# wangbaonan/RAG-SNVBERT

Hardware: AMD Instinct MI355X
Metric: masked SNVs imputed/sec (+ kNN queries/sec), window=1024 k=32 (higher is better)
Workload: dtype bf16

## Files before the change

### include/snvrag.h

```cpp
#ifndef SNVRAG_H
#define SNVRAG_H

#include <stddef.h>
#include <stdint.h>

#ifdef __cplusplus
extern "C" {
#endif

#define SNVRAG_ABI_VERSION 31

enum { SNVRAG_F32 = 0, SNVRAG_BF16 = 1 };
enum { SNVRAG_ACT_NONE = 0, SNVRAG_ACT_GELU = 1, SNVRAG_ACT_LRELU = 2, SNVRAG_ACT_SIGMOID = 3 };

int snvrag_abi_version(void);
const char* snvrag_last_error(void);
int snvrag_device_info(int device, char* name, int name_len);
int snvrag_set_option(const char* name, int64_t value);
int snvrag_get_option(const char* name, int64_t* value);

typedef struct {
  const float* bias;
  const float* row1; int64_t row1_stride; const float* col1;
  const float* row2; int64_t row2_stride; const float* col2;
// ... 61 lines not shown
} snvrag_afgate_w_t;
int snvrag_af_gate(int dtype_out, int64_t M, int64_t D, const float* af, const float* af_p,
                   const snvrag_afgate_w_t* w, void* out, void* stream);

int snvrag_rag_weighted_concat(int dtype, int64_t M, int64_t D, const void* q, const void* rag,
                               const void* wgt, int64_t period, void* out, void* stream);

int snvrag_hap_head_out(int dtype_in, int64_t M, int64_t K, const void* H, int64_t ldh,
                        const float* w , const float* b ,
                        float* logits , float* probs , void* stream);
typedef struct {
  const float* f_w; const float* f_b;
  const float* n_w; const float* n_b;
  const float* w1; const float* b1;
  const float* ln_w; const float* ln_b;
  const float* w2; const float* b2;
  const float* c_w; const float* c_b;
} snvrag_gt_w_t;
int snvrag_gt_head(int64_t M, const float* p1, const float* p2, const float* ref,
                   const float* het, const float* hom, int64_t period,
                   const snvrag_gt_w_t* w, float* out , void* stream);

size_t snvrag_knn_lut_bytes(int64_t nq, int32_t n_sites_pad, int limbs);
int snvrag_knn_lut(int64_t nq, int64_t L, int64_t D, const int64_t* tok_q, const float* W,
                   const float* Aq, int64_t aq_period, const float* Ar,
                   const uint8_t* site_mask, int32_t n_sites, int32_t n_sites_pad,
                   int tok0, int tok1, int mask_tok, int limbs,
                   void* lut_out, int32_t* exp_out, float* const_out, void* stream);
int snvrag_knn_lut_panel(int64_t nq, int64_t L, int64_t D, const int64_t* tok_q, const float* W,
                         const float* Wp, const float* Aq, int64_t aq_period, const float* Ar,
                         const uint8_t* site_mask, int32_t n_sites, int32_t n_sites_pad,
                         int tok0, int tok1, int mask_tok, int limbs,
                         void* lut_out, int32_t* exp_out, float* const_out, void* stream);

int snvrag_knn_scan_parts(int64_t n_ref, int32_t nq);
int snvrag_knn_scan(const uint8_t* codes, int64_t n_ref, int64_t ld_codes, int32_t n_sites_pad,
                    const void* lut, int32_t nq, int limbs, int k, int64_t ref_offset,
                    uint64_t* part_keys, int32_t n_parts, const int32_t* th_init, void* stream);
int snvrag_knn_threshold(const uint64_t* keys, int32_t nq, int k, int32_t* th_out, void* stream);
size_t snvrag_topk_merge_ws_bytes(int32_t n_lists, int32_t nq, int k);
int snvrag_topk_merge(const uint64_t* keys, int32_t n_lists, int32_t nq, int k,
                      uint64_t* out_keys, void* ws, size_t ws_bytes, void* stream);
int snvrag_knn_decode(const uint64_t* keys, int32_t nq, int k, const int32_t* exps,
                      const float* consts, int64_t* idx_out, float* dist_out, void* stream);

int snvrag_knn_emb_splits(int64_t N, int64_t K, int Bq);
size_t snvrag_knn_emb_ws_bytes(int64_t N, int Bq, int splits);
size_t snvrag_knn_emb_packed_bytes(int64_t N, int64_t K);
int snvrag_knn_emb_pack(const void* E, int64_t N, int64_t K, void* Et, void* stream);
int snvrag_knn_emb_scan(const void* Et, int64_t N, int64_t K, const void* Q, int Bq, int splits, float* ws,
                        void* stream);
int snvrag_knn_emb_finish(const float* ws, int splits, int Bq, int64_t N, const float* qn, const float* rn,
                          float* dist, void* stream);

int snvrag_rag_mean(int dtype_out, int64_t nq, int64_t L, int64_t D, int k, const int64_t* idx,
                    const uint8_t* codes, int64_t ld_codes, int32_t n_sites,
                    const float* W, const float* pe, const float* Ar,
                    int tok0, int tok1, int sos, int eos, int pad, void* out, void* stream);

int snvrag_neighbor_counts(int64_t nq, int k, const int64_t* idx, const uint8_t* codes, int64_t ld,
                           int64_t row0, int64_t n_rows, uint8_t* counts, int64_t ld_out, void* stream);
int snvrag_rag_mean_counts(int dtype_out, int64_t nq, int64_t L, int64_t D, int k, const int64_t* idx,
                           const uint8_t* counts, int64_t ld_counts, int32_t n_sites,
                           const float* W, const float* pe, const float* Ar,
                           int tok0, int tok1, int sos, int eos, int pad, void* out, void* stream);

// ... 250 lines not shown
```

### rag-snvbert_amd/csrc/common.h

```cpp
#pragma once
#include <hip/hip_runtime.h>
#include <stdint.h>
#include <stddef.h>
#include <string>
#include <type_traits>

#pragma clang diagnostic ignored "-Winline-asm"

#include "../../include/snvrag.h"
#include "host.h"

namespace snvrag {

typedef __bf16 bf16;
typedef __bf16 bf16x8 __attribute__((ext_vector_type(8)));
typedef __bf16 bf16x4 __attribute__((ext_vector_type(4)));
typedef float f32x4 __attribute__((ext_vector_type(4)));
typedef float f32x16 __attribute__((ext_vector_type(16)));
typedef int i32x4 __attribute__((ext_vector_type(4)));
typedef uint32_t u32x4 __attribute__((ext_vector_type(4)));

void set_error(const std::string& msg);

enum EvKind { EV_GEMM = 1, EV_ATTN = 2, EV_LN = 3, EV_KNN_SCAN = 4, EV_KNN_LUT = 5, EV_MERGE = 6, EV_OTHER = 7, EV_BLOCK = 8,
              EV_ATTN_BWD = 10, EV_TRAIN = 11 };
bool evlog_on();
void evlog_begin(hipStream_t s);
void evlog_end(hipStream_t s, int kind, double work);
struct Options {
  int64_t knn_no_reduce;
  int64_t scan_mode;
  int64_t scan_nt;
  int64_t unfused_ln;
  int64_t encoder_chunk;
  int64_t gemm_tile128;
  int64_t gemm_nw;
  int64_t tail_variant;
  int64_t tail_desync;
  int64_t sg_desync;
  int64_t mlp_desync;
  int64_t g2_desync;
  int64_t sg_waves4;
  int64_t ln_bwd_nopf;
  int64_t attn_variant;
  int64_t dw_xcd;
  int64_t ln_rows1;
  int64_t g2_groups;
  int64_t g2_variant;
  int64_t tail_split;
  int64_t proj_wide;
  int64_t tail_wide;
  int64_t tail_qkv;
  int64_t deterministic;
};
Options& options();
unsigned long long* diag_stamps();

int tailw_launch(int M, const void* att, const void* resid, void* out, const void* ws, const float* vec,
                 const float* b_o, const float* g1, const float* be1, float eps, int desync, int var,
                 const void* pw, const float* pbias, void* qkv_out, hipStream_t s);

int projw_launch(int M, int NC, const void* x, const void* ws, const float* bias, void* out, int desync, hipStream_t s);

// ... 95 lines not shown
```

### rag-snvbert_amd/csrc/knn.hip

```cpp
#include "common.h"

namespace snvrag {

constexpr uint64_t KEY_MAX = ~0ull;
constexpr int KEY_BIAS = 1 << 30;
constexpr int SCAN_CAP = 64;
constexpr int SCAN_TH = SCAN_CAP - 16;

__device__ __forceinline__ uint64_t make_key(int d, uint32_t idx) {
  return ((uint64_t)(uint32_t)(d + KEY_BIAS) << 32) | idx;
}

__device__ __forceinline__ int gcd_u(int a, int b) {
  uint32_t x = (uint32_t)a, y = (uint32_t)b;
  while (y) { const uint32_t t = x % y; x = y; y = t; }
  return (int)x;
}

constexpr int LUT_CH = 64;
__host__ __device__ inline int lut_nch_max(int n_sites_pad) { return 2 * n_sites_pad / LUT_CH + 4; }

__global__ __launch_bounds__(256) void lut_delta_kernel(int L, int D, const int64_t* __restrict__ tok_q,
                                                        const float* __restrict__ W, const float* __restrict__ Wp,
                                                        const float* __restrict__ Aq,
// ... 532 lines not shown
  }
}

__global__ void panel_pack_bits_kernel(const uint8_t* __restrict__ codes, long n, long ld, uint8_t* __restrict__ bits,
                                       long ldb) {
  const long chunks_per_row = ldb / 2;
  const long id = (long)blockIdx.x * blockDim.x + threadIdx.x;
  if (id >= n * chunks_per_row) return;
  const long r = id / chunks_per_row;
  const long c0 = (id % chunks_per_row) * 16;
  uint32_t w = 0;
  if (c0 < ld) {
    const u32x4 v = *reinterpret_cast<const u32x4*>(codes + r * ld + c0);
#pragma unroll
    for (int j = 0; j < 16; ++j) w |= ((v[j >> 2] >> (8 * (j & 3))) & 1u) << j;
  }
  *reinterpret_cast<uint16_t*>(bits + r * ldb + c0 / 8) = (uint16_t)w;
}

__global__ void panel_unpack_rows_kernel(const uint8_t* __restrict__ bits, long n_ref, long ldb,
                                         const int64_t* __restrict__ rows, long n_rows, uint8_t* __restrict__ out,
                                         long ld_out) {
  const long chunks_per_row = ld_out / 16;
  const long id = (long)blockIdx.x * blockDim.x + threadIdx.x;
  if (id >= n_rows * chunks_per_row) return;
  const long i = id / chunks_per_row;
  const long c0 = (id % chunks_per_row) * 16;
  const long r = rows[i];
  u32x4 v = u32x4{0, 0, 0, 0};
  if (r >= 0 && r < n_ref && c0 < 8 * ldb) v = expand16(*reinterpret_cast<const uint16_t*>(bits + r * ldb + c0 / 8));
  *reinterpret_cast<u32x4*>(out + i * ld_out + c0) = v;
}

constexpr int S2_CAP = 64;
constexpr int S2_TH = S2_CAP - 16;
constexpr int S2_LDS = 160 * 1024;
constexpr int S2_CAND = 8 * 16 * S2_CAP * 8;
__host__ __device__ constexpr int s2_rows(int KS) { return 32; }
__host__ __device__ constexpr int s2_nst(int KS) {
  return (S2_LDS - S2_CAND) / (s2_rows(KS) * KS * 64) > 3 ? 3 : (S2_LDS - S2_CAND) / (s2_rows(KS) * KS * 64);
}

template <int PPW, int V>
__device__ __forceinline__ void vm_wait_stages(int y) {
  if constexpr (V <= 0) {
    asm volatile("s_waitcnt vmcnt(0)" ::: "memory");
  } else {
    if (y >= V) {
      asm volatile("s_waitcnt vmcnt(%0)" ::"n"(PPW * V) : "memory");
      return;
    }
    vm_wait_stages<PPW, V - 1>(y);
  }
}
typedef uint32_t u32x2 __attribute__((ext_vector_type(2)));
constexpr int S2B_PD = 3;
#ifndef S2_QTW1
#define S2_QTW1 1
#endif

__device__ __forceinline__ void compact_row2(uint64_t* buf, int row, int cnt, int k, int lane, int& new_cnt,
                                             int& new_th) {
  uint64_t key = lane < cnt ? buf[row * S2_CAP + lane] : KEY_MAX;
  key = wave_sort64(key, lane);
  if (lane < k) buf[row * S2_CAP + lane] = key;
  new_cnt = cnt < k ? cnt : k;
// ... 289 lines not shown
                                    const float* Wp, const float* Aq, int64_t aq_period, const float* Ar,
                                    const uint8_t* site_mask, int32_t n_sites, int32_t n_sites_pad, int tok0,
                                    int tok1, int mask_tok, int limbs, void* lut_out, int32_t* exp_out,
                                    float* const_out, void* stream) {
  SNV_CHECK_PTRS(tok_q, W, Wp, site_mask, lut_out, exp_out);
  SNV_CHECK_ARG(limbs == 1 || limbs == 2, "limbs must be 1 or 2");
  SNV_CHECK_ARG(n_sites_pad % 64 == 0 && n_sites_pad >= n_sites && n_sites + 2 <= L, "site padding");
  SNV_CHECK_ARG(n_sites_pad <= 20 * 64, "window longer than 1280 sites");
  if (nq == 0) return 0;
  hipStream_t s = as_stream(stream);
  const size_t sh = (size_t)(n_sites_pad + 4) * sizeof(float);
  if (limbs == 2) {
    char* tail = (char*)lut_out + lut_tail_offset(nq, n_sites_pad);
    SNV_HIP(hipMemsetAsync(tail, 0, (size_t)((nq + 15) / 16) * 16 * 4 + 16, s));
  }
  float* gdelta = (float*)((char*)lut_out + lut_ws_offset(nq, n_sites_pad, limbs));
  float* gcpart = gdelta + (size_t)nq * n_sites_pad;
  if (Aq || Ar) {
    SNV_CHECK_ARG(D % 4 == 0 && aligned(16, W, Wp, Aq, Ar),
                  "offset LUT: D % 4 == 0 and 16-byte aligned W / Wp / Aq / Ar (float4 rows)");
    const int64_t nch = std::min<int64_t>((L + LUT_CH - 1) / LUT_CH, lut_nch_max(n_sites_pad));
    hipLaunchKernelGGL(lut_delta_kernel, dim3((unsigned)nch, (unsigned)nq), dim3(256), 0, s,
                       (int)L, (int)D, tok_q, W, Wp, Aq, (long)aq_period, Ar, site_mask, n_sites, n_sites_pad, tok0,
                       tok1, mask_tok, gdelta, gcpart);
    SNV_LAUNCH_CHECK();
  }
  hipLaunchKernelGGL(lut_kernel, dim3((unsigned)nq), dim3(256), sh, s, (int)L, (int)D, tok_q, W, Wp, Aq,
                     (long)aq_period, Ar, site_mask, n_sites, n_sites_pad, (int)nq, tok0, tok1, mask_tok,
                     limbs, (int8_t*)lut_out, exp_out, const_out, gdelta, gcpart);
  SNV_LAUNCH_CHECK();
  if (nq % 16)
    hipLaunchKernelGGL(lut_zero_pad_kernel, dim3(64), dim3(256), 0, s, (int8_t*)lut_out, (int)nq,
                       n_sites_pad / 64, limbs);
  SNV_LAUNCH_CHECK();
  return 0;
}

__global__ void threshold_kernel(const uint64_t* __restrict__ keys, int nq, int k, int* __restrict__ th) {
  const int q = blockIdx.x * blockDim.x + threadIdx.x;
  if (q >= nq) return;
  const uint64_t key = keys[(long)q * k + k - 1];
  th[q] = key == KEY_MAX ? INT_MAX : (int)(key >> 32) - KEY_BIAS + 1;
}

extern "C" int snvrag_knn_threshold(const uint64_t* keys, int32_t nq, int k, int32_t* th_out, void* stream) {
  SNV_CHECK_ARG(keys && th_out && k >= 1, "bad arguments");
  if (nq == 0) return 0;
  hipLaunchKernelGGL(threshold_kernel, dim3((nq + 255) / 256), dim3(256), 0, as_stream(stream), keys, (int)nq, k,
                     (int*)th_out);
  SNV_LAUNCH_CHECK();
  return 0;
}

extern "C" int snvrag_knn_scan_parts(int64_t n_ref, int32_t nq) { return scan_parts(n_ref, nq); }

static int scan_check(const char* entry, const void* panel, const void* lut, const uint64_t* part_keys, int limbs,
                      int k, int64_t n_ref, int64_t ref_offset, int32_t n_parts) {
  SNV_CHECK_AS(entry, non_null(panel, lut, part_keys), "null pointer");
  SNV_CHECK_AS(entry, k >= 1 && k <= 32, "k must be in [1, 32]");
  SNV_CHECK_AS(entry, limbs == 1 || limbs == 2, "limbs");
  SNV_CHECK_AS(entry, n_parts >= 1, "n_parts");
  SNV_CHECK_AS(entry, n_ref + ref_offset < (1LL << 32), "panel index must fit 32 bits");
  return 0;
}
struct ScanPlan { long range; const int* wide; };
static ScanPlan scan_plan(int64_t n_ref, int32_t n_parts, int32_t nq, int32_t n_sites_pad, int limbs, const void* lut) {
// ... 263 lines not shown
```

### rag-snvbert_amd/csrc/misc.hip

```cpp
#include "common.h"

#include <cctype>
#include <cstdlib>
#include <cstring>

namespace snvrag {

static thread_local std::string g_err;

struct EvLog {
  bool on = false;
  int cap = 0, n = 0;
  hipEvent_t* ev = nullptr;
  int* kind = nullptr;
  double* work = nullptr;
};
static EvLog g_ev;

bool evlog_on() { return g_ev.on && g_ev.n < g_ev.cap; }
void evlog_begin(hipStream_t s) {
  if (evlog_on()) (void)hipEventRecord(g_ev.ev[2 * g_ev.n], s);
}
void evlog_end(hipStream_t s, int kind, double work) {
  if (!evlog_on()) return;
// ... 43 lines not shown
    }
  }
  {
    f32x4 c = __builtin_amdgcn_mfma_f32_16x16x4f32((float)A[li][lg], (float)B[lg][li], f32x4{0, 0, 0, 0}, 0, 0, 0);
    for (int i = 0; i < 4; ++i) {
      const int row = 4 * lg + i, col = li;
      int ref = 0;
      for (int k = 0; k < 4; ++k) ref += A[row][k] * B[k][col];
      err += c[i] != (float)ref;
    }
  }
  atomicAdd(errors, err);
}

}

using namespace snvrag;

namespace snvrag {
namespace {
struct OptDesc { const char* name; int64_t Options::*field; int64_t dflt; };
const OptDesc kOpts[] = {
    {"knn_no_reduce", &Options::knn_no_reduce, 0}, {"scan_mode", &Options::scan_mode, 0},
    {"scan_nt", &Options::scan_nt, -1},            {"unfused_ln", &Options::unfused_ln, 0},
    {"encoder_chunk", &Options::encoder_chunk, 0}, {"gemm_tile128", &Options::gemm_tile128, 0},
    {"gemm_nw", &Options::gemm_nw, 0},             {"tail_variant", &Options::tail_variant, 0},
    {"tail_desync", &Options::tail_desync, -1},    {"sg_desync", &Options::sg_desync, -1},      {"mlp_desync", &Options::mlp_desync, -1},      {"g2_desync", &Options::g2_desync, -1},
    {"sg_waves4", &Options::sg_waves4, 0},         {"ln_bwd_nopf", &Options::ln_bwd_nopf, 0},
    {"attn_variant", &Options::attn_variant, 0},   {"dw_xcd", &Options::dw_xcd, 1},
    {"ln_rows1", &Options::ln_rows1, 0},           {"tail_wide", &Options::tail_wide, 1},
    {"proj_wide", &Options::proj_wide, 1},         {"g2_variant", &Options::g2_variant, 0},
    {"g2_groups", &Options::g2_groups, 0},         {"tail_split", &Options::tail_split, 64},
    {"deterministic", &Options::deterministic, 0}, {"tail_qkv", &Options::tail_qkv, 1},
};
Options make_options() {
  Options o{};
  for (const OptDesc& d : kOpts) {
    std::string env = "SNVRAG_";
    for (const char* c = d.name; *c; ++c) env += (char)toupper(*c);
    const char* v = getenv(env.c_str());
    o.*(d.field) = v ? atoll(v) : d.dflt;
  }
  return o;
}
const OptDesc* find_opt(const char* name) {
  for (const OptDesc& d : kOpts)
    if (name && strcmp(d.name, name) == 0) return &d;
  return nullptr;
}
}
Options& options() {
  static Options o = make_options();
  return o;
}
}

extern "C" int snvrag_set_option(const char* name, int64_t value) {
  const snvrag::OptDesc* d = snvrag::find_opt(name);
  if (!d) return fail(__func__, std::string("unknown option ") + (name ? name : "(null)"));
  snvrag::options().*(d->field) = value;
  return 0;
}

extern "C" int snvrag_get_option(const char* name, int64_t* value) {
  const snvrag::OptDesc* d = snvrag::find_opt(name);
  if (!d || !value) return fail(__func__, std::string("unknown option ") + (name ? name : "(null)"));
// ... 63 lines not shown
```

### rag-snvbert_amd/src/dataset/embedding_rag_dataset.py

```python

from __future__ import annotations

from collections import OrderedDict, defaultdict
from typing import Dict, List, Optional

import numpy as np
import torch

from ..train_forward import NeighbourGroup
from .dataset import PanelData, TrainDataset, Window
from .utils import mask_probs, sequence_padding
from .vocab import WordVocab

MAX_SEQ_LEN = 1030


class EmbeddingRAGDataset(TrainDataset):
    def __init__(self, vocab, vcf, pos, panel, freq, window, type_to_idx, pop_to_idx, pos_to_idx,
                 ref_gt: Optional[np.ndarray] = None, ref_pos: Optional[np.ndarray] = None,
                 embedding_layer=None, build_ref_data: bool = True, n_gpu: int = 1,
                 maf_mask_percentage: int = 10, use_dynamic_mask: bool = False, name: str = "default",
                 index_cache_bytes: int = 64 << 30, panel_cache: str = "window", panel_codes: str = "u8",
                 ref_vcf_path: Optional[str] = None):
        super().__init__(vocab, vcf, pos, panel, freq, window, type_to_idx, pop_to_idx, pos_to_idx)
# ... 173 lines not shown
    if panel_codes not in ("u8", "bits"):
        raise ValueError("panel_codes must be 'u8' (one byte per site, the default) or 'bits' (bit-packed, "
                         f"an eighth of the HBM); got {panel_codes!r}")
    return panel_codes


def load_ref_panel(path, h5_gt_key: str = "calldata/GT"):
    from .dataset import read_genotypes
    return read_genotypes(path, h5_gt_key)


def bit_rows_of(vg, device):
    if vg is None or vg.any_missing or vg.alt_bits.device != torch.device(device):
        return None
    return vg


def panel_index_of(alleles: np.ndarray, ref_af: np.ndarray, device, shard=None, panel_codes: str = "u8",
                   bit_rows=None, site_rows: Optional[np.ndarray] = None):
    from ..retrieval import PanelIndex
    packed = check_panel_codes(panel_codes) == "bits"
    if bit_rows is not None and site_rows is not None:
        bits, n_hap = bit_rows.alt_bits, bit_rows.alt_bits.shape[0]
        r0, r1 = (0, n_hap) if shard is None else shard.bounds(n_hap)
        return PanelIndex.from_bit_rows(bits[r0:r1], site_rows, ref_af, packed=packed, ref_offset=r0, n_total=n_hap,
                                        n_src_sites=bit_rows.n_sites)
    if shard is None:
        return PanelIndex.from_alleles(alleles, ref_af, device, packed=packed)
    r0, r1 = shard.bounds(alleles.shape[0])
    return PanelIndex.from_alleles(alleles[r0:r1], ref_af, device, ref_offset=r0, n_total=alleles.shape[0],
                                   packed=packed)


def retrieve(ds, batch: dict, embedding_layer, device, k: int, masks: List[np.ndarray],
             dense: bool = False, limbs: int = 2) -> dict:
    from ..engine import engine_for
    from .. import kernels as K
    eng = engine_for(embedding_layer)
    train = embedding_layer.training
    P = eng.packed(allow_train=True)
    dev = torch.device(device)
    h1 = h2d(batch["hap_1"], dev).long()
    h2 = h2d(batch["hap_2"], dev).long()
    af = h2d(batch["af"], dev).float()
    B, L = h1.shape
    D = P.W.shape[1]
    groups = defaultdict(list)
    for i, w in enumerate(batch["window_idx"]):
        groups[int(w)].append(i)
    shard = getattr(ds, "panel_shard", None)
    windows = list(groups)
    if shard is not None:
        from ..retrieval.shards import batch_windows
        windows = batch_windows(windows, shard.group)
    block = None if train else eng.input_block(B, L, dev)
    rag_mean = None if train else block[2 * B:]
    rag_idx = torch.empty(2 * B, k, device=dev, dtype=torch.long)
    rag_groups = []
    dense_out = None
    stale = train and getattr(ds, "panel_cache", "fresh") == "window"
    for w in windows:
        rows = groups.get(w, [])
        new_snap = stale and (ds.jit_cache_win_idx != w or ds._panel_snap is None or ds._panel_snap[0] != w)
        index = ds.panel_index(w, dev)
        rows_t = h2d(torch.tensor(rows, dtype=torch.long), dev)
        tok = torch.cat([h1[rows_t], h2[rows_t]], 0).contiguous()
        n = index.n_sites
        site_mask = h2d(torch.from_numpy(np.ascontiguousarray(masks[w][1:1 + n], np.uint8)), dev)
        ref_af = index.ref_af
        afw = af[rows_t]
        same_memo = []

        def same_af() -> bool:
            if not same_memo:
                same_memo.append(bool(torch.equal(afw, ref_af.unsqueeze(0).expand_as(afw))))
            return same_memo[0]
        counts = uniq = None
        p_drop = embedding_layer.dropout.p if train else 0.0
        with torch.no_grad():
            Ar_emb = eng.af_embedding(ref_af.unsqueeze(0), True).float()[0].contiguous() \
                if P.af is not None else None
            Wp, stale_w = None, False
            if stale:
                wtok = _weights_token(P)
                if new_snap:
                    ds._panel_snap = (w, P.W.detach().float().clone(), Ar_emb, wtok)
                _, W_s, Ar_s, wtok_s = ds._panel_snap
                stale_w = wtok != wtok_s
                if stale_w:
                    Wp, Ar_emb = W_s, Ar_s
            Aq_drop = None
            if p_drop > 0 and len(rows):
                Afull = eng.af_embedding(torch.cat([afw, afw]), True).float() if P.af is not None else 0.0
                e_q = P.W[tok] + P.pe[:L] + Afull
                Aq_drop = (torch.nn.functional.dropout(e_q, p_drop, True) - P.W[tok] - P.pe[:L]).contiguous()
            if shard is not None:
                from ..retrieval.shards import any_rank, kernel_ops, sharded_neighbours
                drop_any = any_rank(p_drop > 0, dev, shard.group)
                exact = P.af is not None and not drop_any and (stale_w or any_rank(not same_af(), dev, shard.group))
                ops = kernel_ops(index, P.W, site_mask, k, limbs,
                                 aq_fn=lambda a: eng.af_embedding(a, True).float().contiguous(),
# ... 81 lines not shown
```

### rag-snvbert_amd/src/kernels.py

```python

from __future__ import annotations

import contextlib

import ctypes as C
from typing import Optional, Sequence, Tuple

import torch

from . import native as N
from .native import check, ptr, stream_ptr

_dt = N.dtype_code


def _c(t: torch.Tensor) -> torch.Tensor:
    if not t.is_contiguous():
        raise ValueError("expected a contiguous tensor")
    return t


def linear(x: torch.Tensor, w: torch.Tensor, bias: Optional[torch.Tensor] = None, *,
           act: int = N.ACT_NONE, slope: float = 0.0,
           row1: Optional[Tuple[torch.Tensor, int, torch.Tensor]] = None,
# ... 248 lines not shown


def gt_head(p1, p2, ref, het, hom, period: int, w: "N.GtW") -> torch.Tensor:
    M = p1.numel() // 2
    out = torch.empty(*p1.shape[:-1], 4, device=p1.device, dtype=torch.float32)
    check(N.lib().snvrag_gt_head(M, ptr(_c(p1)), ptr(_c(p2)), ptr(_c(ref)), ptr(_c(het)), ptr(_c(hom)), period,
                                 C.byref(w), ptr(out), stream_ptr()), "gt_head")
    return out


def knn_lut(tok_q: torch.Tensor, W: torch.Tensor, site_mask: torch.Tensor, n_sites: int, n_sites_pad: int,
            limbs: int = 2, Aq: Optional[torch.Tensor] = None, aq_period: int = 0,
            Ar: Optional[torch.Tensor] = None, tok0: int = 5, tok1: int = 6, mask_tok: int = 4,
            Wp: Optional[torch.Tensor] = None):
    N.require_gpu(tok_q)
    nq, L = tok_q.shape
    D = W.shape[1]
    nbytes = N.lib().snvrag_knn_lut_bytes(nq, n_sites_pad, limbs)
    lut = torch.empty(nbytes, device=tok_q.device, dtype=torch.int8)
    exps = torch.empty(nq, device=tok_q.device, dtype=torch.int32)
    consts = torch.empty(nq, device=tok_q.device, dtype=torch.float32)
    if Wp is not None and Wp is not W:
        assert Wp.shape == W.shape and Wp.dtype == torch.float32
        check(N.lib().snvrag_knn_lut_panel(nq, L, D, ptr(_c(tok_q)), ptr(_c(W)), ptr(_c(Wp)), ptr(Aq), aq_period,
                                           ptr(Ar), ptr(_c(site_mask)), n_sites, n_sites_pad, tok0, tok1, mask_tok,
                                           limbs, ptr(lut), ptr(exps), ptr(consts), stream_ptr()), "knn_lut_panel")
    else:
        check(N.lib().snvrag_knn_lut(nq, L, D, ptr(_c(tok_q)), ptr(_c(W)), ptr(Aq), aq_period, ptr(Ar),
                                     ptr(_c(site_mask)), n_sites, n_sites_pad, tok0, tok1, mask_tok, limbs,
                                     ptr(lut), ptr(exps), ptr(consts), stream_ptr()), "knn_lut")
    return lut, exps, consts


def knn_scan(codes: torch.Tensor, n_sites_pad: int, lut: torch.Tensor, nq: int, limbs: int, k: int,
             ref_offset: int = 0, n_parts: Optional[int] = None, th_init: Optional[torch.Tensor] = None) -> torch.Tensor:
    n_ref, ld = codes.shape
    if n_parts is None:
        n_parts = N.lib().snvrag_knn_scan_parts(n_ref, nq)
    parts = torch.empty(n_parts, nq, k, device=codes.device, dtype=torch.int64)
    if th_init is not None:
        assert th_init.dtype == torch.int32 and th_init.numel() == nq
    check(N.lib().snvrag_knn_scan(ptr(_c(codes)), n_ref, ld, n_sites_pad, ptr(lut), nq, limbs, k, ref_offset,
                                  ptr(parts), n_parts, ptr(th_init), stream_ptr()), "knn_scan")
    return parts


def knn_scan_bits(bits: torch.Tensor, n_sites_pad: int, lut: torch.Tensor, nq: int, limbs: int, k: int,
                  ref_offset: int = 0, n_parts: Optional[int] = None,
                  th_init: Optional[torch.Tensor] = None) -> torch.Tensor:
    assert bits.dtype == torch.uint8 and bits.dim() == 2
    n_ref, ldb = bits.shape
    if n_parts is None:
        n_parts = N.lib().snvrag_knn_scan_parts(n_ref, nq)
    parts = torch.empty(n_parts, nq, k, device=bits.device, dtype=torch.int64)
    if th_init is not None:
        assert th_init.dtype == torch.int32 and th_init.numel() == nq
    check(N.lib().snvrag_knn_scan_bits(ptr(_c(bits)), n_ref, ldb, n_sites_pad, ptr(lut), nq, limbs, k, ref_offset,
                                       ptr(parts), n_parts, ptr(th_init), stream_ptr()), "knn_scan_bits")
    return parts


def knn_threshold(keys: torch.Tensor, k: int) -> torch.Tensor:
    nq = keys.shape[0]
    th = torch.empty(nq, device=keys.device, dtype=torch.int32)
    check(N.lib().snvrag_knn_threshold(ptr(_c(keys)), nq, k, ptr(th), stream_ptr()), "knn_threshold")
    return th
# ... 147 lines not shown
def panel_unpack_rows(bits: torch.Tensor, rows: torch.Tensor, ld_out: Optional[int] = None) -> torch.Tensor:
    N.require_gpu(bits, rows)
    assert bits.dtype == torch.uint8 and bits.dim() == 2 and rows.dtype == torch.int64 and rows.dim() == 1
    n_ref, ldb = bits.shape
    ld_out = ld_out or 8 * ldb
    out = torch.empty(rows.numel(), ld_out, device=bits.device, dtype=torch.uint8)
    check(N.lib().snvrag_panel_unpack_rows(ptr(_c(bits)), n_ref, ldb, ptr(_c(rows)), rows.numel(), ptr(out), ld_out,
                                           stream_ptr()), "panel_unpack_rows")
    return out


def encoder_forward(x: torch.Tensor, layers: Sequence["N.LayerW"], heads: int, ws: torch.Tensor) -> torch.Tensor:
    nseq, L, D = x.shape
    arr = (N.LayerW * len(layers))(*layers)
    check(N.lib().snvrag_encoder_forward(_dt(x.dtype), nseq, L, D, heads, len(layers), arr, ptr(_c(x)),
                                         ptr(ws), ws.numel(), stream_ptr()), "encoder_forward")
    return x


def encoder_ws_bytes(dtype: torch.dtype, nseq: int, L: int, D: int, heads: int) -> int:
    return int(N.lib().snvrag_encoder_ws_bytes(_dt(dtype), nseq, L, D, heads))


def selftest_mfma() -> int:
    return int(N.lib().snvrag_selftest_mfma(stream_ptr()))


def set_option(name: str, value: int) -> int:
    import ctypes
    prev = ctypes.c_int64()
    check(N.lib().snvrag_get_option(name.encode(), ctypes.byref(prev)), "get_option")
    check(N.lib().snvrag_set_option(name.encode(), int(value)), "set_option")
    return int(prev.value)


@contextlib.contextmanager
def option(name: str, value: int):
    prev = set_option(name, value)
    try:
        yield
    finally:
        set_option(name, prev)


_det_ws: dict = {}


def deterministic() -> bool:
    v = C.c_int64()
    check(N.lib().snvrag_get_option(b"deterministic", C.byref(v)), "get_option")
    return bool(v.value)


def _det_workspace(dev: torch.device, nbytes: int) -> torch.Tensor:
    key = (dev.index if dev.index is not None else torch.cuda.current_device(), stream_ptr())
    ws = _det_ws.get(key)
    if ws is None or ws.numel() < nbytes:
        ws = _det_ws[key] = torch.empty(max(int(nbytes), 16), device=dev, dtype=torch.uint8)
    return ws


def attention_train_fwd(qkv: torch.Tensor, nseq: int, L: int, heads: int, dh: int, dropout_p: float = 0.0,
                        seed: int = 0):
    N.require_gpu(qkv)
    assert qkv.dtype == torch.bfloat16
    D = heads * dh
# ... 746 lines not shown
```

### rag-snvbert_amd/src/native.py

```python

from __future__ import annotations

import ctypes as C
import os
from pathlib import Path
from typing import Optional

import torch

PKG_DIR = Path(__file__).resolve().parents[1]
LIB_PATH = Path(os.environ.get("SNVRAG_LIB", PKG_DIR / "lib" / "libsnvrag.so"))

F32, BF16 = 0, 1
ACT_NONE, ACT_GELU, ACT_LRELU, ACT_SIGMOID = 0, 1, 2, 3
ABI_VERSION = 31

vp, i64, i32, f32, sz = C.c_void_p, C.c_int64, C.c_int32, C.c_float, C.c_size_t


class DeriveJob(C.Structure):
    _fields_ = [("kind", i32), ("nparts", i32), ("rows", i64), ("cols", i64), ("dst_ld", i64),
                ("piece0", i64), ("pieces", i64), ("part_rows", i64 * 4), ("rs", i64 * 4), ("cs", i64 * 4),
                ("src", vp * 4), ("dst", vp)]

# ... 46 lines not shown


class LayerW(C.Structure):
    _fields_ = [(n, vp) for n in ("w_qkv", "b_qkv", "w_o", "b_o", "ln1_g", "ln1_b", "w1", "b1",
                                  "lnf_g", "lnf_b", "w2", "b2", "ln2_g", "ln2_b", "w2g", "b2g", "c2g")] + [("q_scale", f32)] + \
        [("ffn_v", vp), ("tail_w", vp), ("qkv_pw", vp), ("qkv_sg", vp)]


_SIGS = {
    "snvrag_abi_version": ([], C.c_int),
    "snvrag_last_error": ([], C.c_char_p),
    "snvrag_device_info": ([C.c_int, C.c_char_p, C.c_int], C.c_int),
    "snvrag_set_option": ([C.c_char_p, i64], C.c_int),
    "snvrag_get_option": ([C.c_char_p, C.POINTER(i64)], C.c_int),
    "snvrag_linear": ([C.c_int, C.c_int, i64, i64, i64, vp, i64, vp, i64, vp, i64, C.POINTER(Epilogue), vp], C.c_int),
    "snvrag_linear_ex": ([C.c_int, C.c_int, i64, i64, i64, vp, i64, vp, i64, vp, i64, C.POINTER(Epilogue),
                          C.POINTER(RowNormS), vp], C.c_int),
    "snvrag_layernorm": ([C.c_int, C.c_int, i64, i64, vp, i64, vp, i64, vp, vp, f32, vp, i64,
                          C.POINTER(LnPost), vp], C.c_int),
    "snvrag_attention": ([C.c_int, i64, i64, C.c_int, C.c_int, vp, i64, vp, i64, f32, vp], C.c_int),
    "snvrag_attention_fallbacks": ([C.c_int], C.c_int),
    "snvrag_af_features": ([C.c_int, i64, vp, vp, C.c_int, vp, vp], C.c_int),
    "snvrag_embed_tokens": ([C.c_int, i64, i64, i64, vp, vp, i64, vp, vp, C.c_int, i64, vp, vp], C.c_int),
    "snvrag_posfeat": ([i64, i64, vp, C.POINTER(PosfeatW), vp, vp], C.c_int),
    "snvrag_af_gate": ([C.c_int, i64, i64, vp, vp, C.POINTER(AfGateW), vp, vp], C.c_int),
    "snvrag_rag_weighted_concat": ([C.c_int, i64, i64, vp, vp, vp, i64, vp, vp], C.c_int),
    "snvrag_hap_head_out": ([C.c_int, i64, i64, vp, i64, vp, vp, vp, vp, vp], C.c_int),
    "snvrag_gt_head": ([i64, vp, vp, vp, vp, vp, i64, C.POINTER(GtW), vp, vp], C.c_int),
    "snvrag_knn_lut_bytes": ([i64, i32, C.c_int], sz),
    "snvrag_knn_lut": ([i64, i64, i64, vp, vp, vp, i64, vp, vp, i32, i32, C.c_int, C.c_int, C.c_int,
                        C.c_int, vp, vp, vp, vp], C.c_int),
    "snvrag_knn_lut_panel": ([i64, i64, i64, vp, vp, vp, vp, i64, vp, vp, i32, i32, C.c_int, C.c_int, C.c_int,
                              C.c_int, vp, vp, vp, vp], C.c_int),
    "snvrag_knn_scan_parts": ([i64, i32], C.c_int),
    "snvrag_knn_scan": ([vp, i64, i64, i32, vp, i32, C.c_int, C.c_int, i64, vp, i32, vp, vp], C.c_int),
    "snvrag_knn_threshold": ([vp, i32, C.c_int, vp, vp], C.c_int),
    "snvrag_topk_merge_ws_bytes": ([i32, i32, C.c_int], sz),
    "snvrag_topk_merge": ([vp, i32, i32, C.c_int, vp, vp, sz, vp], C.c_int),
    "snvrag_knn_decode": ([vp, i32, C.c_int, vp, vp, vp, vp, vp], C.c_int),
    "snvrag_knn_emb_splits": ([i64, i64, C.c_int], C.c_int),
    "snvrag_knn_emb_ws_bytes": ([i64, C.c_int, C.c_int], sz),
    "snvrag_knn_emb_packed_bytes": ([i64, i64], sz),
    "snvrag_knn_emb_pack": ([vp, i64, i64, vp, vp], C.c_int),
    "snvrag_knn_emb_scan": ([vp, i64, i64, vp, C.c_int, C.c_int, vp, vp], C.c_int),
    "snvrag_knn_emb_finish": ([vp, C.c_int, C.c_int, i64, vp, vp, vp, vp], C.c_int),
    "snvrag_rag_mean": ([C.c_int, i64, i64, i64, C.c_int, vp, vp, i64, i32, vp, vp, vp, C.c_int, C.c_int,
                         C.c_int, C.c_int, C.c_int, vp, vp], C.c_int),
    "snvrag_panel_synth": ([vp, i64, i64, i32, vp, C.c_uint64, vp], C.c_int),
    "snvrag_hamming_lists": ([i64, i64, i32, C.c_int, vp, vp, vp, vp], C.c_int),
    "snvrag_hamming_list_count": ([], i32),
    "snvrag_panel_synth_rows": ([vp, i64, i64, i64, i32, vp, C.c_uint64, vp], C.c_int),
    "snvrag_neighbor_counts": ([i64, C.c_int, vp, vp, i64, i64, i64, vp, i64, vp], C.c_int),
    "snvrag_rag_mean_counts": ([C.c_int, i64, i64, i64, C.c_int, vp, vp, i64, i32, vp, vp, vp, C.c_int, C.c_int,
                                C.c_int, C.c_int, C.c_int, vp, vp], C.c_int),
    "snvrag_panel_pack_bits": ([vp, i64, i64, vp, i64, vp], C.c_int),
    "snvrag_panel_synth_bits": ([vp, i64, i64, i64, i32, vp, C.c_uint64, vp], C.c_int),
    "snvrag_panel_unpack_rows": ([vp, i64, i64, vp, i64, vp, i64, vp], C.c_int),
    "snvrag_knn_scan_bits": ([vp, i64, i64, i32, vp, i32, C.c_int, C.c_int, i64, vp, i32, vp, vp], C.c_int),
    "snvrag_rag_mean_bits": ([C.c_int, i64, i64, i64, C.c_int, vp, vp, i64, i32, vp, vp, vp, C.c_int, C.c_int,
                              C.c_int, C.c_int, C.c_int, vp, vp], C.c_int),
    "snvrag_neighbor_counts_bits": ([i64, C.c_int, vp, vp, i64, i64, i64, vp, i64, vp], C.c_int),
    "snvrag_encoder_ws_bytes": ([C.c_int, i64, i64, C.c_int, C.c_int], sz),
    "snvrag_encoder_forward": ([C.c_int, i64, i64, C.c_int, C.c_int, C.c_int, C.POINTER(LayerW), vp, vp, sz, vp],
                               C.c_int),
    "snvrag_proj_pack_bytes": ([C.c_int, C.c_int], sz),
    "snvrag_proj_pack": ([C.c_int, C.c_int, vp, vp, vp], C.c_int),
# ... 149 lines not shown
```

### rag-snvbert_amd/src/retrieval/panel_index.py

```python

from __future__ import annotations

import os
from typing import Optional

import numpy as np
import torch

from .. import kernels as K


def pad_sites(n_sites: int) -> int:
    return max(256, ((n_sites + 255) // 256) * 256)


class PanelIndex:
    def __init__(self, codes: torch.Tensor, n_sites: int, ref_af: torch.Tensor, ref_offset: int = 0,
                 n_total: Optional[int] = None, packed: bool = False):
        if codes.dtype != torch.uint8 or codes.dim() != 2:
            raise ValueError("codes must be uint8 [n_ref, ld]" if not packed else "bits must be uint8 [n_ref, ld / 8]")
        self.packed = bool(packed)
        self.bits = codes if self.packed else None
        self._codes = None if self.packed else codes
        self.n_ref = codes.shape[0]
        self.ld = codes.shape[1] * (8 if self.packed else 1)
        self.n_sites = int(n_sites)
        self.n_sites_pad = pad_sites(n_sites)
        if self.ld < self.n_sites_pad:
            raise ValueError("codes row shorter than padded window")
        self.ref_af = ref_af
        self.ref_offset = int(ref_offset)
        self.n_total = int(n_total if n_total is not None else self.n_ref + ref_offset)

    @property
    def codes(self) -> torch.Tensor:
        if self.packed:
            raise AttributeError("a packed PanelIndex holds bits, not u8 codes: gather the rows you need with "
                                 "rows(idx) (kernels.panel_unpack_rows) — nothing unpacks the whole panel")
        return self._codes

    @property
    def data(self) -> torch.Tensor:
        return self.bits if self.packed else self._codes

    @property
    def device(self) -> torch.device:
        return self.data.device

    @classmethod
    def from_alleles(cls, alleles: np.ndarray, ref_af: np.ndarray, device, ref_offset: int = 0,
                     n_total: Optional[int] = None, packed: bool = False) -> "PanelIndex":
        a = np.asarray(alleles)
        if a.size and (a.min() < 0 or a.max() > 1):
            raise ValueError("panel index supports biallelic 0/1 genotypes (got values outside {0,1}); "
                             "binarise multi-allelic/missing calls first")
        n_ref, n_sites = a.shape
        ld = pad_sites(n_sites)
        codes = np.zeros((n_ref, ld), np.uint8)
        codes[:, :n_sites] = a
        if packed:
            bits = np.packbits(codes, axis=1, bitorder="little")
            return cls(torch.from_numpy(bits).to(device), n_sites,
                       torch.as_tensor(np.asarray(ref_af, np.float32), device=device), ref_offset, n_total,
                       packed=True)
        return cls(torch.from_numpy(codes).to(device), n_sites,
# ... 10 lines not shown
                   n_total, packed=packed)

    @classmethod
    def synthetic(cls, n_ref: int, n_sites: int, site_af: torch.Tensor, ref_af: torch.Tensor,
                  seed: int, packed: bool = False) -> "PanelIndex":
        if packed:
            return cls(K.panel_synth_bits(n_ref, n_sites, site_af.float().contiguous(), seed), n_sites, ref_af,
                       packed=True)
        codes = K.panel_synth(n_ref, n_sites, site_af.float().contiguous(), seed)
        return cls(codes, n_sites, ref_af)

    def pack(self) -> "PanelIndex":
        if self.packed:
            return self
        return PanelIndex(K.panel_pack_bits(self._codes), self.n_sites, self.ref_af, self.ref_offset, self.n_total,
                          packed=True)

    @property
    def nbytes(self) -> int:
        return self.data.numel()

    def rows(self, idx: torch.Tensor) -> torch.Tensor:
        if self.packed:
            return K.panel_unpack_rows(self.bits, idx.long().contiguous())
        return self._codes[idx]

    def rag_mean(self, idx: torch.Tensor, W, pe, Ar, L: int, dtype, out=None, counts=None) -> torch.Tensor:
        return K.rag_mean(idx, self.data, self.n_sites, W, pe, Ar, L, dtype, out=out, counts=counts,
                          bits=self.packed)

    def neighbor_counts(self, idx: torch.Tensor) -> torch.Tensor:
        return K.neighbor_counts(idx, self.data, self.ref_offset, bits=self.packed)

    def lut(self, tok_q: torch.Tensor, W: torch.Tensor, site_mask: torch.Tensor, limbs: int = 2,
            Aq: Optional[torch.Tensor] = None, aq_period: int = 0, Ar: Optional[torch.Tensor] = None,
            Wp: Optional[torch.Tensor] = None):
        return K.knn_lut(tok_q.long().contiguous(), W, site_mask, self.n_sites, self.n_sites_pad, limbs,
                         Aq, aq_period, Ar, Wp=Wp)

    SAMPLE_MIN = 1 << 17

    def scan_keys(self, lut: torch.Tensor, nq: int, limbs: int, k: int, presample: Optional[bool] = None) -> torch.Tensor:
        n_ref = self.n_ref
        scan = K.knn_scan_bits if self.packed else K.knn_scan
        data = self.data
        if presample is None:
            presample = n_ref >= self.SAMPLE_MIN
        th = None
        if presample:
            div = int(os.environ.get("SNVRAG_SAMPLE_DIV", "64"))
            rpp = int(os.environ.get("SNVRAG_SAMPLE_RPP", "64"))
            m = max(16 * k, ((n_ref // div) + 15) // 16 * 16)
            sample = scan(data[:m], self.n_sites_pad, lut, nq, limbs, k, self.ref_offset,
                          n_parts=max(1, min(256, m // rpp)))
            th = K.knn_threshold(K.topk_merge(sample, k), k)
        parts = scan(data, self.n_sites_pad, lut, nq, limbs, k, self.ref_offset, th_init=th)
        return K.topk_merge(parts, k)

    def search(self, tok_q: torch.Tensor, W: torch.Tensor, site_mask: torch.Tensor, k: int, limbs: int = 2,
               Aq: Optional[torch.Tensor] = None, aq_period: int = 0, Ar: Optional[torch.Tensor] = None,
               return_keys: bool = False, Wp: Optional[torch.Tensor] = None):
        nq = tok_q.shape[0]
        lut, exps, consts = self.lut(tok_q, W, site_mask, limbs, Aq, aq_period, Ar, Wp=Wp)
        keys = self.scan_keys(lut, nq, limbs, k)
        idx, dist = K.knn_decode(keys, exps, consts)
        if return_keys:
            return idx, dist, keys, lut, exps
        return idx, dist
```

Baseline: 8.054 million.

## Compact panel codes and LUT to unmasked sites before kNN scan

Adds GPU kernels that gather only the unmasked site columns of the reference panel and the matching LUT entries into a narrower padded layout. The kNN scan then runs over the compacted width, so masked sites no longer cost bandwidth or compute. The compacted panel is cached per mask object and version, and the device site mask is cached per window to avoid repeated host-to-device copies. The trade-off is an extra gather pass each time the mask changes, plus extra memory for the compacted panel copy.

After: 8.097 million (median of 6 runs). No clear change (+0.5%).

```diff
diff --git a/include/snvrag.h b/include/snvrag.h
--- a/include/snvrag.h
+++ b/include/snvrag.h
@@ -117,6 +117,12 @@
                          const uint8_t* site_mask, int32_t n_sites, int32_t n_sites_pad,
                          int tok0, int tok1, int mask_tok, int limbs,
                          void* lut_out, int32_t* exp_out, float* const_out, void* stream);
+
+int snvrag_panel_compact(const uint8_t* codes, int64_t n_ref, int64_t ld, int32_t n_cols,
+                         const int32_t* site_list, int32_t n_c, uint8_t* out, int64_t ldc, void* stream);
+size_t snvrag_knn_lut_compact_bytes(int64_t nq, int32_t ldc, int limbs);
+int snvrag_knn_lut_compact(const void* lut, int64_t nq, int32_t n_sites_pad, int limbs,
+                           const int32_t* site_list, int32_t n_c, int32_t ldc, void* out, void* stream);
 
 int snvrag_knn_scan_parts(int64_t n_ref, int32_t nq);
 int snvrag_knn_scan(const uint8_t* codes, int64_t n_ref, int64_t ld_codes, int32_t n_sites_pad,
diff --git a/rag-snvbert_amd/csrc/common.h b/rag-snvbert_amd/csrc/common.h
--- a/rag-snvbert_amd/csrc/common.h
+++ b/rag-snvbert_amd/csrc/common.h
@@ -29,6 +29,7 @@
 void evlog_end(hipStream_t s, int kind, double work);
 struct Options {
   int64_t knn_no_reduce;
+  int64_t knn_compact;
   int64_t scan_mode;
   int64_t scan_nt;
   int64_t unfused_ln;
diff --git a/rag-snvbert_amd/csrc/knn.hip b/rag-snvbert_amd/csrc/knn.hip
--- a/rag-snvbert_amd/csrc/knn.hip
+++ b/rag-snvbert_amd/csrc/knn.hip
@@ -588,6 +588,65 @@
   *reinterpret_cast<u32x4*>(out + i * ld_out + c0) = v;
 }
 
+constexpr int PC_ROWS = 16, PC_MAXLD = 1280;
+__global__ __launch_bounds__(256) void panel_compact_kernel(const uint8_t* __restrict__ codes, long n_ref, long ld,
+                                                            int n_cols, const int* __restrict__ site_list, int n_c,
+                                                            uint8_t* __restrict__ out, long ldc) {
+  __shared__ __attribute__((aligned(16))) uint8_t srow[PC_ROWS * PC_MAXLD];
+  __shared__ int ssite[PC_MAXLD];
+  const int tid = threadIdx.x;
+  for (int j = tid; j < ldc; j += 256) {
+    const int s = j < n_c ? site_list[j] : -1;
+    ssite[j] = (unsigned)s < (unsigned)n_cols ? s : -1;
+  }
+  const int cpr = n_cols / 16, opr = (int)(ldc / 16);
+  for (long r0 = (long)blockIdx.x * PC_ROWS; r0 < n_ref; r0 += (long)gridDim.x * PC_ROWS) {
+    const int nr = (int)min((long)PC_ROWS, n_ref - r0);
+    __syncthreads();
+    for (int id = tid; id < nr * cpr; id += 256) {
+      const int row = id / cpr, c = id % cpr;
+      *reinterpret_cast<u32x4*>(srow + row * n_cols + 16 * c) =
+          *reinterpret_cast<const u32x4*>(codes + (r0 + row) * ld + 16 * c);
+    }
+    __syncthreads();
+    for (int id = tid; id < nr * opr; id += 256) {
+      const int row = id / opr, c = id % opr;
+      u32x4 v = u32x4{0, 0, 0, 0};
+#pragma unroll
+      for (int e = 0; e < 16; ++e) {
+        const int s = ssite[16 * c + e];
+        const uint32_t b = s >= 0 ? srow[row * n_cols + s] : 0u;
+        v[e >> 2] |= b << (8 * (e & 3));
+      }
+      *reinterpret_cast<u32x4*>(out + (r0 + row) * ldc + 16 * c) = v;
+    }
+  }
+}
+
+__global__ __launch_bounds__(256) void lut_compact_kernel(const int8_t* __restrict__ lut, int nq, int KS, int limbs,
+                                                          const int* __restrict__ site_list, int n_c, int KSc,
+                                                          int8_t* __restrict__ out) {
+  const int qt = blockIdx.x, p = blockIdx.y, tid = threadIdx.x;
+  const long nqt = (nq + 15) >> 4;
+  const long src_plane = p < limbs ? (long)qt * limbs + p : nqt * 2 + qt;
+  const int8_t* src = lut + src_plane * KS * 1024;
+  int8_t* dst = out + src_plane * KSc * 1024;
+  for (int i = tid; i < KSc * 1024; i += 256) {
+    const int b = i & 15, lane = (i >> 4) & 63, ks = i >> 10;
+    const int j = ks * 64 + (lane >> 4) * 16 + b, qr = lane & 15;
+    const int s = j < n_c ? site_list[j] : -1;
+    int8_t v = 0;
+    if ((unsigned)s < (unsigned)(KS * 64)) v = src[(((s >> 6) * 64 + ((s & 63) >> 4) * 16 + qr) << 4) + (s & 15)];
+    dst[i] = v;
+  }
+  if (limbs == 2 && p == 0) {
+    const int* mult = reinterpret_cast<const int*>(lut + nqt * 3 * KS * 1024);
+    int* multc = reinterpret_cast<int*>(out + nqt * 3 * KSc * 1024);
+    if (tid < 16) multc[qt * 16 + tid] = mult[qt * 16 + tid];
+    if (qt == 0 && tid == 16) multc[nqt * 16] = mult[nqt * 16];
+  }
+}
+
 constexpr int S2_CAP = 64;
 constexpr int S2_TH = S2_CAP - 16;
 constexpr int S2_LDS = 160 * 1024;
@@ -943,6 +1002,55 @@
   if (nq % 16)
     hipLaunchKernelGGL(lut_zero_pad_kernel, dim3(64), dim3(256), 0, s, (int8_t*)lut_out, (int)nq,
                        n_sites_pad / 64, limbs);
+  SNV_LAUNCH_CHECK();
+  return 0;
+}
+
+static int panel_compact_check(const char* entry, const uint8_t* codes, int64_t n_ref, int64_t ld, int32_t n_cols,
+                               const int32_t* site_list, int32_t n_c, const uint8_t* out, int64_t ldc) {
+  SNV_CHECK_AS(entry, non_null(codes, site_list, out), "null pointer");
+  SNV_CHECK_AS(entry, ld % 16 == 0 && aligned(16, codes, out), "codes and out must be 16-byte aligned rows");
+  SNV_CHECK_AS(entry, n_ref >= 0 && n_cols >= 16 && n_cols % 16 == 0 && n_cols <= ld && n_cols <= PC_MAXLD,
+               "n_cols: a multiple of 16 up to min(ld, 1280)");
+  SNV_CHECK_AS(entry, ldc >= 256 && ldc % 256 == 0 && ldc <= PC_MAXLD && n_c >= 0 && n_c <= ldc && aligned(4, site_list),
+               "ldc a multiple of 256 up to 1280, 0 <= n_c <= ldc");
+  return 0;
+}
+
+extern "C" int snvrag_panel_compact(const uint8_t* codes, int64_t n_ref, int64_t ld, int32_t n_cols,
+                                    const int32_t* site_list, int32_t n_c, uint8_t* out, int64_t ldc, void* stream) {
+  if (int rc = panel_compact_check(__func__, codes, n_ref, ld, n_cols, site_list, n_c, out, ldc)) return rc;
+  if (n_ref == 0) return 0;
+  hipStream_t s = as_stream(stream);
+  const int grid = (int)std::min<long>(cdiv(n_ref, PC_ROWS), 8L * cu_count());
+  evlog_begin(s);
+  hipLaunchKernelGGL(panel_compact_kernel, dim3(grid), dim3(256), 0, s, codes, (long)n_ref, (long)ld, (int)n_cols,
+                     site_list, (int)n_c, out, (long)ldc);
+  SNV_LAUNCH_CHECK();
+  evlog_end(s, EV_OTHER, (double)n_ref * ((double)n_cols + (double)ldc));
+  return 0;
+}
+
+extern "C" size_t snvrag_knn_lut_compact_bytes(int64_t nq, int32_t ldc, int limbs) { return lut_ws_offset(nq, ldc, limbs); }
+
+static int lut_compact_check(const char* entry, const void* lut, int64_t nq, int32_t n_sites_pad, int limbs,
+                             const int32_t* site_list, int32_t n_c, int32_t ldc, const void* out) {
+  SNV_CHECK_AS(entry, non_null(lut, site_list, out), "null pointer");
+  SNV_CHECK_AS(entry, limbs == 1 || limbs == 2, "limbs must be 1 or 2");
+  SNV_CHECK_AS(entry, nq >= 0 && n_sites_pad % 64 == 0 && n_sites_pad >= 64 && n_sites_pad <= 20 * 64, "site padding");
+  SNV_CHECK_AS(entry, ldc >= 256 && ldc % 256 == 0 && ldc <= 20 * 64 && n_c >= 0 && n_c <= ldc,
+               "ldc a multiple of 256 up to 1280, 0 <= n_c <= ldc");
+  SNV_CHECK_AS(entry, aligned(4, lut, site_list, out), "lut, site_list and out must be 4-byte aligned");
+  return 0;
+}
+
+extern "C" int snvrag_knn_lut_compact(const void* lut, int64_t nq, int32_t n_sites_pad, int limbs,
+                                      const int32_t* site_list, int32_t n_c, int32_t ldc, void* out, void* stream) {
+  if (int rc = lut_compact_check(__func__, lut, nq, n_sites_pad, limbs, site_list, n_c, ldc, out)) return rc;
+  if (nq == 0) return 0;
+  hipLaunchKernelGGL(lut_compact_kernel, dim3((unsigned)((nq + 15) / 16), limbs == 2 ? 3 : 1), dim3(256), 0,
+                     as_stream(stream), (const int8_t*)lut, (int)nq, n_sites_pad / 64, limbs, site_list, (int)n_c,
+                     ldc / 64, (int8_t*)out);
   SNV_LAUNCH_CHECK();
   return 0;
 }
diff --git a/rag-snvbert_amd/csrc/misc.hip b/rag-snvbert_amd/csrc/misc.hip
--- a/rag-snvbert_amd/csrc/misc.hip
+++ b/rag-snvbert_amd/csrc/misc.hip
@@ -99,6 +99,7 @@
     {"proj_wide", &Options::proj_wide, 1},         {"g2_variant", &Options::g2_variant, 0},
     {"g2_groups", &Options::g2_groups, 0},         {"tail_split", &Options::tail_split, 64},
     {"deterministic", &Options::deterministic, 0}, {"tail_qkv", &Options::tail_qkv, 1},
+    {"knn_compact", &Options::knn_compact, 1},
 };
 Options make_options() {
   Options o{};
diff --git a/rag-snvbert_amd/src/dataset/embedding_rag_dataset.py b/rag-snvbert_amd/src/dataset/embedding_rag_dataset.py
--- a/rag-snvbert_amd/src/dataset/embedding_rag_dataset.py
+++ b/rag-snvbert_amd/src/dataset/embedding_rag_dataset.py
@@ -229,6 +229,14 @@
                                    packed=packed)
 
 
+def _site_mask_on(ds, w: int, mask: np.ndarray, n: int, dev: torch.device) -> torch.Tensor:
+    cache = ds.__dict__.setdefault("_site_mask_dev", {})
+    ent = cache.get((w, str(dev)))
+    if ent is None or ent[0] is not mask or ent[1].numel() != n:
+        ent = cache[(w, str(dev))] = (mask,h2d(torch.from_numpy(np.ascontiguousarray(mask[1:1 + n], np.uint8)), dev))
+    return ent[1]
+
+
 def retrieve(ds, batch: dict, embedding_layer, device, k: int, masks: List[np.ndarray],
              dense: bool = False, limbs: int = 2) -> dict:
     from ..engine import engine_for
@@ -263,7 +271,7 @@
         rows_t = h2d(torch.tensor(rows, dtype=torch.long), dev)
         tok = torch.cat([h1[rows_t], h2[rows_t]], 0).contiguous()
         n = index.n_sites
-        site_mask = h2d(torch.from_numpy(np.ascontiguousarray(masks[w][1:1 + n], np.uint8)), dev)
+        site_mask = _site_mask_on(ds, w, masks[w], n, dev)
         ref_af = index.ref_af
         afw = af[rows_t]
         same_memo = []
diff --git a/rag-snvbert_amd/src/kernels.py b/rag-snvbert_amd/src/kernels.py
--- a/rag-snvbert_amd/src/kernels.py
+++ b/rag-snvbert_amd/src/kernels.py
@@ -304,6 +304,30 @@
     return lut, exps, consts
 
 
+def knn_lut_compact(lut: torch.Tensor, nq: int, n_sites_pad: int, limbs: int, site_list: torch.Tensor,
+                    ldc: int) -> torch.Tensor:
+    assert site_list.dtype == torch.int32 and site_list.device == lut.device
+    out = torch.empty(N.lib().snvrag_knn_lut_compact_bytes(nq, ldc, limbs), device=lut.device, dtype=torch.int8)
+    check(N.lib().snvrag_knn_lut_compact(ptr(_c(lut)), nq, n_sites_pad, limbs, ptr(_c(site_list)), site_list.numel(),
+                                         ldc, ptr(out), stream_ptr()), "knn_lut_compact")
+    return out
+
+
+def panel_compact(codes: torch.Tensor, n_cols: int, site_list: torch.Tensor, ldc: int,
+                  out: Optional[torch.Tensor] = None) -> torch.Tensor:
+    N.require_gpu(codes)
+    assert codes.dtype == torch.uint8 and codes.dim() == 2 and codes.stride(1) == 1
+    assert site_list.dtype == torch.int32 and site_list.device == codes.device
+    n_ref = codes.shape[0]
+    ld = max(codes.stride(0), codes.shape[1])
+    if out is None:
+        out = torch.empty(n_ref, ldc, device=codes.device, dtype=torch.uint8)
+    assert out.dtype == torch.uint8 and out.is_contiguous() and out.shape[0] >= n_ref and out.shape[1] == ldc
+    check(N.lib().snvrag_panel_compact(ptr(codes), n_ref, ld, n_cols, ptr(_c(site_list)), site_list.numel(),
+                                       ptr(out), ldc, stream_ptr()), "panel_compact")
+    return out
+
+
 def knn_scan(codes: torch.Tensor, n_sites_pad: int, lut: torch.Tensor, nq: int, limbs: int, k: int,
              ref_offset: int = 0, n_parts: Optional[int] = None, th_init: Optional[torch.Tensor] = None) -> torch.Tensor:
     n_ref, ld = codes.shape
@@ -517,6 +541,12 @@
     check(N.lib().snvrag_get_option(name.encode(), ctypes.byref(prev)), "get_option")
     check(N.lib().snvrag_set_option(name.encode(), int(value)), "set_option")
     return int(prev.value)
+
+
+def get_option(name: str) -> int:
+    v = C.c_int64()
+    check(N.lib().snvrag_get_option(name.encode(), C.byref(v)), "get_option")
+    return int(v.value)
 
 
 @contextlib.contextmanager
diff --git a/rag-snvbert_amd/src/native.py b/rag-snvbert_amd/src/native.py
--- a/rag-snvbert_amd/src/native.py
+++ b/rag-snvbert_amd/src/native.py
@@ -102,6 +102,9 @@
                         C.c_int, vp, vp, vp, vp], C.c_int),
     "snvrag_knn_lut_panel": ([i64, i64, i64, vp, vp, vp, vp, i64, vp, vp, i32, i32, C.c_int, C.c_int, C.c_int,
                               C.c_int, vp, vp, vp, vp], C.c_int),
+    "snvrag_panel_compact": ([vp, i64, i64, i32, vp, i32, vp, i64, vp], C.c_int),
+    "snvrag_knn_lut_compact_bytes": ([i64, i32, C.c_int], sz),
+    "snvrag_knn_lut_compact": ([vp, i64, i32, C.c_int, vp, i32, i32, vp, vp], C.c_int),
     "snvrag_knn_scan_parts": ([i64, i32], C.c_int),
     "snvrag_knn_scan": ([vp, i64, i64, i32, vp, i32, C.c_int, C.c_int, i64, vp, i32, vp, vp], C.c_int),
     "snvrag_knn_threshold": ([vp, i32, C.c_int, vp, vp], C.c_int),
diff --git a/rag-snvbert_amd/src/retrieval/panel_index.py b/rag-snvbert_amd/src/retrieval/panel_index.py
--- a/rag-snvbert_amd/src/retrieval/panel_index.py
+++ b/rag-snvbert_amd/src/retrieval/panel_index.py
@@ -12,6 +12,14 @@
 
 def pad_sites(n_sites: int) -> int:
     return max(256, ((n_sites + 255) // 256) * 256)
+
+
+class _MaskView:
+    __slots__ = ("mask", "version", "sites", "n_c", "ldc", "codes")
+
+    def __init__(self, mask: torch.Tensor, version: int, sites: torch.Tensor, ldc: int):
+        self.mask, self.version, self.sites, self.n_c, self.ldc = mask, version, sites, sites.numel(), ldc
+        self.codes: Optional[torch.Tensor] = None
 
 
 class PanelIndex:
@@ -31,6 +39,8 @@
         self.ref_af = ref_af
         self.ref_offset = int(ref_offset)
         self.n_total = int(n_total if n_total is not None else self.n_ref + ref_offset)
+        self._view: Optional[_MaskView] = None
+        self.compact_builds = 0
 
     @property
     def codes(self) -> torch.Tensor:
@@ -107,18 +117,44 @@
     def neighbor_counts(self, idx: torch.Tensor) -> torch.Tensor:
         return K.neighbor_counts(idx, self.data, self.ref_offset, bits=self.packed)
 
+    def _mask_view(self, site_mask: torch.Tensor) -> Optional["_MaskView"]:
+        if self.packed or not K.get_option("knn_compact"):
+            return None
+        v = self._view
+        if v is None or v.mask is not site_mask or v.version != site_mask._version:
+            sites = torch.nonzero(site_mask[:self.n_sites] == 0).flatten().to(torch.int32)
+            v = self._view = _MaskView(site_mask, site_mask._version, sites, pad_sites(sites.numel()))
+        return v if 1 <= v.n_c and v.ldc < self.n_sites_pad else None
+
+    def _compact_codes(self, v: "_MaskView") -> torch.Tensor:
+        mine = self._view
+        if mine is None or mine.mask is not v.mask or mine.version != v.version:
+            mine = self._view = _MaskView(v.mask, v.version, v.sites, v.ldc)
+        if mine.codes is None:
+            mine.codes = K.panel_compact(self._codes, self.n_sites_pad, mine.sites, mine.ldc)
+            self.compact_builds += 1
+        return mine.codes
+
     def lut(self, tok_q: torch.Tensor, W: torch.Tensor, site_mask: torch.Tensor, limbs: int = 2,
             Aq: Optional[torch.Tensor] = None, aq_period: int = 0, Ar: Optional[torch.Tensor] = None,
             Wp: Optional[torch.Tensor] = None):
-        return K.knn_lut(tok_q.long().contiguous(), W, site_mask, self.n_sites, self.n_sites_pad, limbs,
-                         Aq, aq_period, Ar, Wp=Wp)
+        lut, exps, consts = K.knn_lut(tok_q.long().contiguous(), W, site_mask, self.n_sites, self.n_sites_pad, limbs,
+                                      Aq, aq_period, Ar, Wp=Wp)
+        v = self._mask_view(site_mask)
+        if v is not None:
+            lut.compact = (v, K.knn_lut_compact(lut, tok_q.shape[0], self.n_sites_pad, limbs, v.sites, v.ldc))
+        return lut, exps, consts
 
     SAMPLE_MIN = 1 << 17
 
     def scan_keys(self, lut: torch.Tensor, nq: int, limbs: int, k: int, presample: Optional[bool] = None) -> torch.Tensor:
         n_ref = self.n_ref
         scan = K.knn_scan_bits if self.packed else K.knn_scan
-        data = self.data
+        data, row = self.data, self.n_sites_pad
+        tag = getattr(lut, "compact", None)
+        if tag is not None and not self.packed and K.get_option("knn_compact"):
+            v, lut = tag
+            data, row = self._compact_codes(v), v.ldc
         if presample is None:
             presample = n_ref >= self.SAMPLE_MIN
         th = None
@@ -126,10 +162,10 @@
             div = int(os.environ.get("SNVRAG_SAMPLE_DIV", "64"))
             rpp = int(os.environ.get("SNVRAG_SAMPLE_RPP", "64"))
             m = max(16 * k, ((n_ref // div) + 15) // 16 * 16)
-            sample = scan(data[:m], self.n_sites_pad, lut, nq, limbs, k, self.ref_offset,
+            sample = scan(data[:m], row, lut, nq, limbs, k, self.ref_offset,
                           n_parts=max(1, min(256, m // rpp)))
             th = K.knn_threshold(K.topk_merge(sample, k), k)
-        parts = scan(data, self.n_sites_pad, lut, nq, limbs, k, self.ref_offset, th_init=th)
+        parts = scan(data, row, lut, nq, limbs, k, self.ref_offset, th_init=th)
         return K.topk_merge(parts, k)
 
     def search(self, tok_q: torch.Tensor, W: torch.Tensor, site_mask: torch.Tensor, k: int, limbs: int = 2,
```
